# Circuitscape/Circuitscape.jl

Hardware: AMD Instinct MI355X
Metric: pair-solves/sec (AMG-PCG, setup amortised over 100 pairs) on 10000x10000 raster pairwise (higher is better)
Workload: dtype f64

## Files before the change

### circuitscape.jl_amd/csrc/common.h

```cpp
#pragma once
#include <hip/hip_runtime.h>

#include <atomic>
#include <cstdint>
#include <cstdlib>
#include <map>
#include <mutex>
#include <cstdio>
#include <cstring>
#include <stdexcept>
#include <string>
#include <utility>
#include <vector>

#include "../../include/csgpu.h"

namespace csgpu {

struct Error : public std::runtime_error {
  int code;
  Error(int c, const std::string& m) : std::runtime_error(m), code(c) {}
};

#define CS_HIP(expr)                                                                                    \
  do {                                                                                                  \
    hipError_t _e = (expr);                                                                             \
    if (_e != hipSuccess) {                                                                             \
      char _buf[512];                                                                                   \
      snprintf(_buf, sizeof(_buf), "%s failed: %s (%s:%d)", #expr, hipGetErrorString(_e), __FILE__,     \
               __LINE__);                                                                               \
      throw ::csgpu::Error((int)_e == (int)hipErrorOutOfMemory ? CSGPU_OOM : CSGPU_HIP_ERROR, _buf);    \
    }                                                                                                   \
  } while (0)

#define CS_REQUIRE(cond, code, msg)                  \
  do {                                               \
    if (!(cond)) throw ::csgpu::Error((code), (msg)); \
  } while (0)

inline void check_launch(const char* what) {
  hipError_t e = hipGetLastError();
  if (e != hipSuccess) throw Error(CSGPU_HIP_ERROR, std::string(what) + ": " + hipGetErrorString(e));
}

struct Knobs {
  int last_level_sweeps = 0;
  bool enrich = true;
  int enrich_steps = 6;
  double enrich_tau = 0.06;
  int64_t dia25_min_rows = 16384;
  bool dia25_prefetch = true;
  int dia25_waves = 0;
  bool dia25_fused_j0 = true;
  int stream = 0;
  int64_t stream_min = (int64_t)1 << 25;
  double hetero_fp64_frac = 0.03;
  int tail_rows = 4096;
  int poly_lattice = 0;
  double poly_strength = 0.0, poly_coef = 1.0, poly_smin = 8.0, poly_smax = 1000.0;
  bool cellspace = true, cellspace_from_csr = true;
  double cellspace_min_frac = 0.5;
  bool lattice_l1 = true;
  int lattice_l1_min_rows = 16384;
  bool stencil = true, two_product = true;
  bool direct_lattice = true, lattice_s = true, lattice_q = true, direct_tiles = true, tile_pieces = true, direct_at = true;
  double tile_theta = 0.03, tile_split_min = 0.005;
  bool dirichlet_coarse = true, deflation = true, tail_projection = true;
  bool expander_probe = true;
  bool reorder = false;
  int coarse_smoother = 0;
  int nu_l1 = 0, nu_deep = 0;
  int64_t host_stream_block = 0;
  bool wide_csr = false;
  bool fixed_k = false;
  bool recompute_ap = true;
  int fused_restrict = 0;
  int fused_seg = 64;
  int fused_level1 = 0;
  bool sparse_init = true;
  int64_t collapse_min = -1;
  bool longrow = true, narrow_tile = false;
  int spmv_grid_cap = 65536, dia_seg = 0, restrict_seg = 32;
  int verbose = 0;
  double pinv_cut = 0.0;
  bool kernel_gain_ref = false, tail_debug = false;
  bool galerkin_staged = false;
  bool raster_transpose = true;
  bool enrich_fused = true;
  int apq_nt = 256;
  int timed_launches = 512;
};

inline const Knobs*& knobs_slot() {
  static thread_local const Knobs* p = nullptr;
  return p;
}
inline const Knobs& knobs() {
  static const Knobs dflt;
  const Knobs* p = knobs_slot();
  return p ? *p : dflt;
}
struct KnobScope {
  const Knobs* prev;
  explicit KnobScope(const Knobs* k) : prev(knobs_slot()) { knobs_slot() = k; }
  ~KnobScope() { knobs_slot() = prev; }
  KnobScope(const KnobScope&) = delete;
  KnobScope& operator=(const KnobScope&) = delete;
};

static std::atomic<int64_t> g_live_bytes{0};

struct DevicePool {
  static const int kMaxDev = 64;
  struct Blk {
    void* p;
    size_t cap;
    uint64_t seq;
  };
  std::mutex mu[kMaxDev];
  std::multimap<size_t, Blk> ready[kMaxDev];
  std::vector<Blk> pending[kMaxDev];
  size_t pooled[kMaxDev] = {0};
  size_t limit[kMaxDev] = {0};
  std::atomic<uint64_t> seq{0};
  bool enabled = getenv("CSGPU_NO_POOL") == nullptr;
  void promote(int dev) {
    if (pending[dev].empty()) return;
    (void)hipDeviceSynchronize();
    for (const Blk& b : pending[dev]) ready[dev].emplace(b.cap, b);
    pending[dev].clear();
  }
  void* take(int dev, size_t b, size_t* cap) {
    std::lock_guard<std::mutex> lk(mu[dev]);
    for (int pass = 0; pass < 2; ++pass) {
      auto it = ready[dev].lower_bound(b);
      if (it != ready[dev].end() && it->first <= b + b / 8) {
        void* p = it->second.p;
        *cap = it->second.cap;
        ready[dev].erase(it);
        pooled[dev] -= *cap;
        return p;
      }
      if (pass == 0) {
        bool fits = false;
        for (const Blk& q : pending[dev]) fits = fits || (q.cap >= b && q.cap <= b + b / 8);
        if (!fits) break;
        promote(dev);
      }
    }
    return nullptr;
  }
  void give(int dev, size_t cap, void* p) {
    std::vector<void*> victims;
    {
      std::lock_guard<std::mutex> lk(mu[dev]);
      if (limit[dev] == 0) {
        size_t fr = 0, tot = 0;
        const char* e = getenv("CSGPU_POOL_MAX_GB");
        if (e) limit[dev] = (size_t)(atof(e) * 1073741824.0) + 1;
        else {
          int cur = dev;
          (void)hipGetDevice(&cur);
          if (cur != dev) (void)hipSetDevice(dev);
          const bool ok = hipMemGetInfo(&fr, &tot) == hipSuccess && tot > 0;
          if (cur != dev) (void)hipSetDevice(cur);
          limit[dev] = ok ? tot / 10 * 6 : (size_t)64 << 30;
        }
      }
      pending[dev].push_back(Blk{p, cap, ++seq});
      pooled[dev] += cap;
      if (pooled[dev] > limit[dev]) {
        int cur = dev;
        (void)hipGetDevice(&cur);
        if (cur != dev) (void)hipSetDevice(dev);
        promote(dev);
        if (cur != dev) (void)hipSetDevice(cur);
        while (pooled[dev] > limit[dev] && !ready[dev].empty()) {
          auto oldest = ready[dev].begin();
          for (auto it = ready[dev].begin(); it != ready[dev].end(); ++it)
            if (it->second.seq < oldest->second.seq) oldest = it;
          victims.push_back(oldest->second.p);
          pooled[dev] -= oldest->second.cap;
          ready[dev].erase(oldest);
        }
      }
    }
    for (void* v : victims) hipFree(v);
  }
  size_t trim(int dev) {
    size_t freed = 0;
    for (int d = 0; d < kMaxDev; ++d) {
      if (dev >= 0 && d != dev) continue;
      std::vector<void*> victims;
      {
        std::lock_guard<std::mutex> lk(mu[d]);
        for (auto& kv : ready[d]) victims.push_back(kv.second.p);
        for (const Blk& b : pending[d]) victims.push_back(b.p);
        freed += pooled[d];
        ready[d].clear();
        pending[d].clear();
        pooled[d] = 0;
      }
      for (void* p : victims) hipFree(p);
    }
    return freed;
  }
};
inline DevicePool& device_pool() {
  static DevicePool* p = new DevicePool();
  return *p;
}

struct DBuf {
  void* p = nullptr;
  size_t bytes = 0;
  size_t cap = 0;
  int dev = -1;
  DBuf() {}
  explicit DBuf(size_t b) { alloc(b); }
  DBuf(const DBuf&) = delete;
  DBuf& operator=(const DBuf&) = delete;
  DBuf(DBuf&& o) noexcept : p(o.p), bytes(o.bytes), cap(o.cap), dev(o.dev) {
    o.p = nullptr;
    o.bytes = 0;
    o.cap = 0;
  }
  DBuf& operator=(DBuf&& o) noexcept {
    if (this != &o) {
      release();
      p = o.p;
      bytes = o.bytes;
      cap = o.cap;
      dev = o.dev;
      o.p = nullptr;
      o.bytes = 0;
      o.cap = 0;
    }
    return *this;
  }
  ~DBuf() { release(); }
  void alloc(size_t b) {
    release();
    if (b == 0) return;
    CS_HIP(hipGetDevice(&dev));
    DevicePool& pool = device_pool();
    const bool poolable = pool.enabled && dev >= 0 && dev < DevicePool::kMaxDev;
    cap = b;
    if (poolable) p = pool.take(dev, b, &cap);
    if (!p) {
      cap = b;
      hipError_t e = hipMalloc(&p, b);
      if (e != hipSuccess && poolable && pool.trim(dev) > 0) {
        (void)hipGetLastError();
        e = hipMalloc(&p, b);
      }
      if (e != hipSuccess) {
        p = nullptr;
        cap = 0;
        CS_HIP(e);
      }
    }
    bytes = b;
    g_live_bytes += (int64_t)b;
  }
  void release() {
    if (p) {
      DevicePool& pool = device_pool();
      if (pool.enabled && dev >= 0 && dev < DevicePool::kMaxDev)
        pool.give(dev, cap, p);
      else
        hipFree(p);
      g_live_bytes -= (int64_t)bytes;
    }
    p = nullptr;
    bytes = 0;
    cap = 0;
  }
  template <class U>
  U* as() const {
    return (U*)p;
  }
};

template <class U>
inline U* dptr(const DBuf& b) {
  return (U*)b.p;
}

template <class U>
inline DBuf dalloc(size_t count) {
  return DBuf(count * sizeof(U));
}

template <class T>
struct Csr {
  int nrows = 0, ncols = 0;
  int64_t nnz = 0;
  DBuf rowptr, col, val;
  const int* rp() const { return rowptr.as<int>(); }
  const int* ci() const { return col.as<int>(); }
  const T* va() const { return val.as<T>(); }
  int* rp() { return rowptr.as<int>(); }
  int* ci() { return col.as<int>(); }
  T* va() { return val.as<T>(); }
  size_t device_bytes() const { return rowptr.bytes + col.bytes + val.bytes; }
};

template <class T>
struct Dia {
  int64_t n = 0;
  int R = 0;
  DBuf rows;
  const T* data() const { return rows.as<T>(); }
  size_t device_bytes() const { return rows.bytes; }
};

template <class T>
struct LatticeQ {
  int64_t n = 0;
  int R = 0, C = 0, Rc = 0, Cc = 0;
  DBuf q;
  const T* data() const { return q.as<T>(); }
  size_t device_bytes() const { return q.bytes; }
};

inline int ceil_div(int64_t a, int64_t b) { return (int)((a + b - 1) / b); }

static const int kBlock = 256;
static const int kMaxGrid = 2048;
inline int grid_for(int64_t work_items, int per_block = kBlock) {
  int64_t g = (work_items + per_block - 1) / per_block;
  if (g < 1) g = 1;
  if (g > kMaxGrid) g = kMaxGrid;
  return (int)g;
}

}
```

### circuitscape.jl_amd/csrc/csgpu.hip

```cpp
#include <atomic>
#include <chrono>
#include <memory>
#include <mutex>
#include <thread>

#include "currents.h"
#include "pairs.h"
#include "pcg.h"
#include "raster.h"
#include "lattice_setup.h"
#include "reorder.h"

namespace csgpu {

static thread_local std::string g_last_error;

struct GroundedJob {
  const void* rhs = nullptr;
  const int64_t *sptr = nullptr, *sidx = nullptr;
  const void* sval = nullptr;
  const int64_t *gptr = nullptr, *gidx = nullptr;
  const int64_t* check = nullptr;
  void *check_out = nullptr, *x_out = nullptr, *curr_out = nullptr, *cum_inout = nullptr, *max_inout = nullptr;
};
// ... 834 lines not shown
    if (ok) {
      amg_setup_levels(H, sp, nullptr, nullptr, carry, st);
      CS_HIP(hipEventRecord(e1, st));
      CS_HIP(hipEventSynchronize(e1));
      float ms = 0;
      CS_HIP(hipEventElapsedTime(&ms, e0, e1));
      H.setup_ms = ms;
      if constexpr (MIXED) Aouter.nrows = Aouter.ncols = (int)n;
      csr_ready = false;
      if (kn.verbose)
        fprintf(stderr, "csgpu: %lld x %lld raster through the index-free pipeline (%lld rows, %lld nodes, %d levels)\n",
                (long long)R, (long long)C, (long long)n, (long long)n_api, (int)H.levels.size());
    }
    hipEventDestroy(e0);
    hipEventDestroy(e1);
    return ok;
  }

  bool setup_lattice_direct(DBuf& dcond, DBuf& dground, DBuf& node, int64_t R, int64_t C, int four, int avg_res, int reg,
                            std::chrono::steady_clock::time_point t0, int colmajor = 0) {
    const int64_t ncells = R * C;
    const int gc = grid_for(ncells);
    if (cellspace) {
      cellmap.alloc((size_t)ncells * sizeof(int));
      node2cell.alloc((size_t)n_api * sizeof(int));
      cell2node.alloc((size_t)ncells * sizeof(int));
    }
    hipLaunchKernelGGL((raster_maps_kernel<T>), dim3(gc), dim3(256), 0, st, (int)R, (int)C, (const T*)dptr<T>(dcond),
                       (const int*)dptr<int>(node), dptr<int>(nodemap), cellspace ? dptr<int>(cellmap) : (int*)nullptr,
                       cellspace ? dptr<int>(node2cell) : (int*)nullptr, cellspace ? dptr<int>(cell2node) : (int*)nullptr,
                       colmajor);
    dia.n = ncells;
    dia.R = (int)R;
    dia.rows.alloc((size_t)ncells * 5 * sizeof(T));
    if (dground.p) ground_node.alloc((size_t)ncells * sizeof(T));
    DBuf part = dalloc<double>(gc), cnt = dalloc<unsigned long long>(gc), size0;
    hipLaunchKernelGGL((raster_dia_kernel<T>), dim3(gc), dim3(256), 0, st, (int)R, (int)C, four, avg_res,
                       (const T*)dptr<T>(dcond), dground.p ? (const T*)dptr<T>(dground) : (const T*)nullptr, dptr<T>(dia.rows),
                       dground.p ? dptr<T>(ground_node) : (T*)nullptr, dptr<double>(part), dptr<unsigned long long>(cnt),
                       colmajor);
    if (cellspace) size0.alloc((size_t)ncells * sizeof(long long));
    hipLaunchKernelGGL((raster_dia_finish_kernel<T>), dim3(gc), dim3(256), 0, st, (int)R, (int)C, (const T*)dptr<T>(dcond),
                       dptr<T>(dia.rows), (const double*)dptr<double>(part), gc,
                       reg ? (double)std::numeric_limits<T>::epsilon() : 0.0,
                       cellspace ? dptr<long long>(size0) : (long long*)nullptr, colmajor);
    std::vector<unsigned long long> hc((size_t)gc);
    CS_HIP(hipMemcpyAsync(hc.data(), cnt.p, hc.size() * sizeof(unsigned long long), hipMemcpyDeviceToHost, st));
    check_launch("raster -> lattice form");
    CS_HIP(hipStreamSynchronize(st));
    nnz_api = 0;
    for (unsigned long long v : hc) nnz_api += (int64_t)v;
    nnz = nnz_api + (n - n_api);
    dcond.release();
    dground.release();
    node.release();
    upload_ms = std::chrono::duration<double, std::milli>(std::chrono::steady_clock::now() - t0).count();
    if (lattice_pipeline_hierarchy(size0, R, C)) return true;
    CS_REQUIRE(nnz < ((int64_t)1 << 31), CSGPU_BAD_ARGS, "raster too large for the CSR pipeline");
    Csr<T> A;
    dia_to_csr(dia, A, st);
    DBuf drow((size_t)n * sizeof(int)), dcol((size_t)n * sizeof(int));
    hipLaunchKernelGGL(lattice_coords_kernel, dim3(grid_for(n)), dim3(256), 0, st, n, (int)R, dptr<int>(drow), dptr<int>(dcol));
    dia = Dia<T>();
    finish_setup(std::move(A), dptr<int>(drow), dptr<int>(dcol), (int)R,
                 cellspace ? (const long long*)dptr<long long>(size0) : (const long long*)nullptr);
    return true;
  }

  void setup_from_raster(const void* cond, int64_t R, int64_t C, int four, int avg_res, int reg,
                         const void* ground = nullptr) {
    KnobScope ks(&kn);
    auto t0 = std::chrono::steady_clock::now();
    const int64_t ncells = R * C;
    DBuf dcond((size_t)ncells * sizeof(T));
    CS_HIP(hipMemcpyAsync(dcond.p, cond, (size_t)ncells * sizeof(T), hipMemcpyHostToDevice, st));
    DBuf dground;
    if (ground) {
      dground.alloc((size_t)ncells * sizeof(T));
      CS_HIP(hipMemcpyAsync(dground.p, ground, (size_t)ncells * sizeof(T), hipMemcpyHostToDevice, st));
    }
    DBuf node = dalloc<int>((size_t)ncells + 1);
    CS_HIP(hipMemsetAsync(node.p, 0, ((size_t)ncells + 1) * sizeof(int), st));
    const int gc = grid_for(ncells);
    const bool transposed = kn.raster_transpose && R >= 32 && C >= 32;
    DBuf dcondT, dgroundT;
    if (transposed) {
      const int gt = (int)std::min<int64_t>(((R + 31) / 32) * ((C + 31) / 32), 65536);
      dcondT.alloc((size_t)ncells * sizeof(T));
      hipLaunchKernelGGL((raster_transpose_kernel<T>), dim3(gt), dim3(256), 0, st, (int)R, (int)C, (const T*)dptr<T>(dcond),
                         dptr<T>(dcondT));
      if (ground) {
        dgroundT.alloc((size_t)ncells * sizeof(T));
        hipLaunchKernelGGL((raster_transpose_kernel<T>), dim3(gt), dim3(256), 0, st, (int)R, (int)C,
                           (const T*)dptr<T>(dground), dptr<T>(dgroundT));
      }
    }
    hipLaunchKernelGGL((raster_valid_kernel<T>), dim3(gc), dim3(256), 0, st, (int)R, (int)C,
                       transposed ? dptr<T>(dcondT) : dptr<T>(dcond), dptr<int>(node), transposed ? 1 : 0);
    DBuf total = dalloc<int>(1);
    exclusive_scan_i32(dptr<int>(node), ncells + 1, st, dptr<int>(total));
    n_api = read_int(dptr<int>(total), st);
    CS_REQUIRE(n_api > 0, CSGPU_BAD_ARGS, "raster has no cell with positive conductance");
    cellspace = want_cellspace(n_api, ncells, R, C);
    n = cellspace ? ncells : n_api;
    raster_rows = R;
    raster_cols = C;
    nodemap.alloc((size_t)ncells * sizeof(int));
    if (n == ncells && want_lattice_pipeline(R, C)) {
      if (setup_lattice_direct(transposed ? dcondT : dcond, transposed ? dgroundT : dground, node, R, C, four, avg_res, reg, t0,
                               transposed ? 1 : 0))
        return;
    }
    CS_REQUIRE(ncells * 9 < ((int64_t)1 << 31), CSGPU_BAD_ARGS,
               "raster too large for the CSR pipeline (int32 entry offsets); only all-valid / mostly-valid rasters without "
               "polygons, with the default two-product fine level, go through the index-free pipeline");
    if (cellspace) {
      cellmap.alloc((size_t)ncells * sizeof(int));
      node2cell.alloc((size_t)n_api * sizeof(int));
      cell2node.alloc((size_t)ncells * sizeof(int));
    }
    Csr<T> A;
    A.nrows = A.ncols = (int)n;
    A.rowptr.alloc((size_t)(n + 1) * sizeof(int));
    CS_HIP(hipMemsetAsync(A.rp(), 0, (size_t)(n + 1) * sizeof(int), st));
    hipLaunchKernelGGL((raster_count_kernel<T>), dim3(gc), dim3(256), 0, st, (int)R, (int)C, four, dptr<T>(dcond),
                       dptr<int>(node), A.rp(), dptr<int>(nodemap), cellspace ? 1 : 0,
                       cellspace ? dptr<int>(cellmap) : (int*)nullptr, cellspace ? dptr<int>(node2cell) : (int*)nullptr,
                       cellspace ? dptr<int>(cell2node) : (int*)nullptr);
    exclusive_scan_i32(A.rp(), n + 1, st, dptr<int>(total));
    nnz = read_int(dptr<int>(total), st);
    nnz_api = nnz - (n - n_api);
    A.nnz = nnz;
    A.col.alloc((size_t)nnz * sizeof(int));
    A.val.alloc((size_t)nnz * sizeof(T));
    DBuf drow((size_t)n * sizeof(int)), dcol((size_t)n * sizeof(int));
    if (ground) ground_node.alloc((size_t)n * sizeof(T));
    hipLaunchKernelGGL((raster_fill_kernel<T>), dim3(gc), dim3(256), 0, st, (int)R, (int)C, four, avg_res,
                       dptr<T>(dcond), dptr<int>(node), A.rp(), A.ci(), A.va(), dptr<int>(drow), dptr<int>(dcol),
                       ground ? (const T*)dptr<T>(dground) : (const T*)nullptr,
                       ground ? dptr<T>(ground_node) : (T*)nullptr, cellspace ? 1 : 0);
    if (reg) {
      const int g = grid_for(nnz);
      DBuf part = dalloc<double>(g);
      hipLaunchKernelGGL((dot_kernel<T, 1, false>), dim3(g), dim3(256), 0, st, nnz, (const T*)A.va(), (const T*)A.va(),
                         dptr<double>(part), (const T*)nullptr, (const T*)nullptr, (double*)nullptr);
      hipLaunchKernelGGL((add_scalar_kernel<T>), dim3(g), dim3(256), 0, st, nnz, A.va(), dptr<double>(part), g,
                         (double)std::numeric_limits<T>::epsilon());
      CS_HIP(hipStreamSynchronize(st));
    }
    DBuf size0;
    if (cellspace) {
      size0.alloc((size_t)n * sizeof(long long));
      hipLaunchKernelGGL((raster_identity_kernel<T>), dim3(gc), dim3(256), 0, st, (int)R, (int)C, (const T*)dptr<T>(dcond),
                         (const int*)A.rp(), A.va(), dptr<long long>(size0));
    }
    check_launch("raster build");
    CS_HIP(hipStreamSynchronize(st));
    dcond.release();
    node.release();
    upload_ms = std::chrono::duration<double, std::milli>(std::chrono::steady_clock::now() - t0).count();
    finish_setup(std::move(A), dptr<int>(drow), dptr<int>(dcol), n == ncells ? (int)R : -1,
                 cellspace ? (const long long*)dptr<long long>(size0) : (const long long*)nullptr);
    if (cellspace && !(dia.n > 0 && H.levels[0].lattice_two_product()) && kn.verbose)
      fprintf(stderr, "csgpu: cell-space raster without the index-free fine level (CSR kernels on %lld rows)\n", (long long)n);
  }

  bool setup_poly_lattice(const void* cond, const int32_t* polymap, int64_t R, int64_t C, int four, int avg_res, int reg,
                          bool is_fallback) {
    if (is_fallback || kn.poly_lattice < 0 || !want_lattice_pipeline(R, C)) return false;
    if (!kn.cellspace || ground_node.p) return false;
    auto t0 = std::chrono::steady_clock::now();
    const int64_t ncells = R * C;
    const T* hc = (const T*)cond;
    int32_t maxid = 0;
    for (int64_t k = 0; k < ncells; ++k) maxid = std::max(maxid, polymap[k]);
// ... 2003 lines not shown
                        const void* source_val, const int64_t* ground_ptr, const int64_t* ground_idx,
                        const int64_t* check_node, void* check_out, void* x_out, void* curr_out, void* cum_curr_inout,
                        void* max_curr_inout, csgpu_stats* stats) {
  if (!h || !sources_args_ok(nrhs, source_ptr, source_idx, ground_ptr, ground_idx, check_node, check_out)) {
    g_last_error = "bad arguments";
    return CSGPU_BAD_ARGS;
  }
  csgpu::GroundedJob job;
  job.sptr = source_ptr;
  job.sidx = source_idx;
  job.sval = source_val;
  job.gptr = ground_ptr;
  job.gidx = ground_idx;
  job.check = check_node;
  job.check_out = check_out;
  job.x_out = x_out;
  job.curr_out = curr_out;
  job.cum_inout = cum_curr_inout;
  job.max_inout = max_curr_inout;
  return grounded_call(h, job, nrhs, stats);
}

int csgpu_spmv_bench(csgpu_handle* h, int k, int reps, double* avg_ms) {
  CS_API_BEGIN
  if (!h || !avg_ms || reps < 1 || !(k == 1 || k == 2 || k == 4 || k == 8 || k == 16 || k == 32)) {
    g_last_error = "bad arguments";
    return CSGPU_BAD_ARGS;
  }
  *avg_ms = h->solver->spmv_bench(k, reps);
  return CSGPU_OK;
  CS_API_END
}

int csgpu_spmv_host(csgpu_handle* h, const void* x, void* y, int k) {
  CS_API_BEGIN
  if (!h || !x || !y || !(k == 1 || k == 2 || k == 4 || k == 8 || k == 16 || k == 32)) {
    g_last_error = "bad arguments";
    return CSGPU_BAD_ARGS;
  }
  h->solver->spmv_host(x, y, k);
  return CSGPU_OK;
  CS_API_END
}

int csgpu_level_spmv_host(csgpu_handle* h, int lvl, int which, const void* x, void* y, int k, double* dots) {
  CS_API_BEGIN
  if (!h || !x || !y || which < 0 || which > 6 || !(k == 1 || k == 2 || k == 4 || k == 8 || k == 16 || k == 32)) {
    g_last_error = "bad arguments";
    return CSGPU_BAD_ARGS;
  }
  h->solver->level_spmv_host(lvl, which, x, y, k, dots);
  return CSGPU_OK;
  CS_API_END
}

int csgpu_get_level_matrix(const csgpu_handle* h, int lvl, int which, int64_t* nrows, int64_t* ncols, int64_t* nnz,
                           int32_t* rowptr, int32_t* colidx, void* vals) {
  CS_API_BEGIN
  if (!h || which < 0 || which > 5) {
    g_last_error = "bad arguments";
    return CSGPU_BAD_ARGS;
  }
  h->solver->get_level_matrix(lvl, which, nrows, ncols, nnz, rowptr, colidx, vals);
  return CSGPU_OK;
  CS_API_END
}

int csgpu_dia_product_host(csgpu_handle* h, const void* z, const void* p_in, const double* beta, void* p_out, void* y,
                           int k, double* dots) {
  CS_API_BEGIN
  if (!h || !z || !p_in || !beta || !p_out || !y || !(k == 1 || k == 2 || k == 4 || k == 8 || k == 16 || k == 32)) {
    g_last_error = "bad arguments";
    return CSGPU_BAD_ARGS;
  }
  h->solver->dia_product_host(z, p_in, beta, p_out, y, k, dots);
  return CSGPU_OK;
  CS_API_END
}

void csgpu_free(csgpu_handle* h) { delete h; }

int64_t csgpu_trim_memory(int device) { return (int64_t)csgpu::device_pool().trim(device); }

}

struct csgpu_multi {
  std::vector<csgpu_handle*> handles;
  std::vector<int> devices;
  int val_bytes = 8;
  int batch = 8;
  std::vector<double> busy_s;
  std::vector<int64_t> pairs_done;
  ~csgpu_multi() {
    for (csgpu_handle* h : handles) delete h;
  }
};

namespace {

int multi_devices(const int32_t* devices, int ndevices, std::vector<int>& out) {
  const int visible = csgpu_device_count();
  if (visible < 1) {
    g_last_error = "no HIP device visible";
    return CSGPU_HIP_ERROR;
  }
  out.clear();
  if (devices) {
    for (int i = 0; i < ndevices; ++i) {
      if (devices[i] < 0 || devices[i] >= visible) {
        g_last_error = "device ordinal out of range";
        return CSGPU_BAD_ARGS;
      }
      out.push_back(devices[i]);
    }
  } else {
    const int nd = ndevices <= 0 ? visible : std::min(ndevices, visible);
    for (int i = 0; i < nd; ++i) out.push_back(i);
  }
  if (out.empty()) {
    g_last_error = "empty device list";
    return CSGPU_BAD_ARGS;
  }
  return CSGPU_OK;
}

template <class F>
int multi_build(const csgpu_opts* opts, const int32_t* devices, int ndevices, int val_bytes, csgpu_multi** out, F build) {
  std::vector<int> devs;
  int rc = multi_devices(devices, ndevices, devs);
  if (rc) return rc;
  std::unique_ptr<csgpu_multi> m(new csgpu_multi());
  m->devices = devs;
  m->val_bytes = val_bytes;
  csgpu_opts o;
  if (opts) o = *opts; else csgpu_default_opts(&o);
  m->batch = std::max(1, std::min(o.batch, (int)csgpu::kMaxK));
  m->handles.assign(devs.size(), nullptr);
  m->busy_s.assign(devs.size(), 0.0);
  m->pairs_done.assign(devs.size(), 0);
  std::vector<int> codes(devs.size(), CSGPU_OK);
  std::vector<std::string> msgs(devs.size());
  std::vector<std::thread> th;
  for (size_t i = 0; i < devs.size(); ++i)
    th.emplace_back([&, i] {
      csgpu_opts oi = o;
      oi.device = devs[i];
      codes[i] = build(&oi, &m->handles[i]);
      if (codes[i]) msgs[i] = csgpu_last_error();
    });
  for (auto& t : th) t.join();
  for (size_t i = 0; i < devs.size(); ++i)
    if (codes[i]) {
      g_last_error = "device " + std::to_string(devs[i]) + ": " + msgs[i];
      return codes[i];
    }
  *out = m.release();
  return CSGPU_OK;
}

void multi_combine_maps(size_t nd, int64_t n, size_t vb, const std::vector<std::vector<char>>& cum,
                        const std::vector<std::vector<char>>& mx, void* cum_curr_inout, void* max_curr_inout) {
  auto combine = [&](int64_t lo, int64_t hi) {
    for (size_t i = 0; i < nd; ++i) {
      if (cum_curr_inout && !cum[i].empty()) {
        if (vb == 8) {
          double* o = (double*)cum_curr_inout;
// ... 395 lines not shown
```

### circuitscape.jl_amd/lib.py

```python
import ctypes
import os

import numpy as np

_HERE = os.path.dirname(os.path.abspath(__file__))
DEFAULT_LIB = os.path.join(_HERE, "libcsgpu.so")

CSGPU_OK, CSGPU_NOT_CONVERGED, CSGPU_HIP_ERROR, CSGPU_OOM, CSGPU_BAD_ARGS, CSGPU_INTERNAL = range(6)
CRIT_KRYLOV, CRIT_TRUE_RESIDUAL, CRIT_BOTH = 0, 1, 2
AGG_AUTO, AGG_MIS2, AGG_GRID = 0, 1, 2

EXPORTS = [
    "csgpu_device_count", "csgpu_default_opts", "csgpu_setup", "csgpu_raster_setup", "csgpu_get_info",
    "csgpu_solve_pairs", "csgpu_solve_pairs_currents", "csgpu_solve_rhs", "csgpu_solve_grounded", "csgpu_solve_sources", "csgpu_solve_region_pairs", "csgpu_spmv_bench", "csgpu_spmv_host", "csgpu_level_spmv_host",
    "csgpu_get_level_matrix", "csgpu_get_permutation", "csgpu_raster_nodemap", "csgpu_components", "csgpu_raster_setup_grounded", "csgpu_raster_setup_poly",
    "csgpu_solve_raster", "csgpu_dia_product_host",
    "csgpu_multi_setup", "csgpu_multi_raster_setup", "csgpu_multi_solve_pairs", "csgpu_multi_solve_pairs_currents",
    "csgpu_multi_solve_grounded", "csgpu_multi_solve_sources", "csgpu_multi_device_count",
    "csgpu_multi_handle", "csgpu_multi_last_busy", "csgpu_multi_free",
    "csgpu_free", "csgpu_trim_memory", "csgpu_last_error", "csgpu_version",
]


class CsgpuError(RuntimeError):
    def __init__(self, code, msg):
        super().__init__(msg)
        self.code = code


OPTS_INT_FIELDS = ("last_level_sweeps", "enrich", "enrich_steps", "dia25_min_rows", "dia25_prefetch", "dia25_waves",
                   "dia25_fused_j0", "stream", "tail_rows", "poly_lattice", "cellspace", "cellspace_from_csr", "lattice_level1",
                   "lattice_level1_min_rows", "lattice_setup", "lattice_s", "lattice_q", "direct_tiles", "tile_pieces",
                   "direct_at", "dirichlet_coarse", "deflation", "tail_projection", "coarse_smoother", "nu_l1", "nu_deep",
                   "wide_csr", "fixed_k", "recompute_ap", "longrow", "narrow_tile", "spmv_grid_cap", "dia_seg", "restrict_seg",
                   "collapse_min", "verbose", "expander_probe", "fused_restrict", "sparse_init", "fused_level1")
OPTS_DOUBLE_FIELDS = ("enrich_tau", "hetero_fp64_frac", "poly_strength", "poly_coef", "poly_smin", "poly_smax",
                      "cellspace_min_frac", "tile_theta", "tile_split_min")


class Opts(ctypes.Structure):
    _fields_ = [
        ("struct_size", ctypes.c_int32), ("device", ctypes.c_int32), ("max_levels", ctypes.c_int32),
        ("max_coarse", ctypes.c_int32), ("aggregation", ctypes.c_int32), ("nu_pre", ctypes.c_int32),
        ("nu_post", ctypes.c_int32), ("criterion", ctypes.c_int32), ("itmax", ctypes.c_int32),
        ("batch", ctypes.c_int32), ("check_every", ctypes.c_int32), ("nu_coarse", ctypes.c_int32),
        ("theta", ctypes.c_double), ("omega_p", ctypes.c_double), ("omega_s", ctypes.c_double),
        ("rtol", ctypes.c_double), ("atol", ctypes.c_double),
        ("node_row", ctypes.c_void_p), ("node_col", ctypes.c_void_p),
        ("precond_bytes", ctypes.c_int32), ("use_graph", ctypes.c_int32),
        ("two_product", ctypes.c_int32), ("stencil", ctypes.c_int32),
        ("explicit_check", ctypes.c_int32), ("reorder", ctypes.c_int32),
    ] + [(name, ctypes.c_int32) for name in OPTS_INT_FIELDS] + [
        ("stream_min", ctypes.c_int64), ("host_stream_block", ctypes.c_int64),
    ] + [(name, ctypes.c_double) for name in OPTS_DOUBLE_FIELDS]


class Info(ctypes.Structure):
    _fields_ = [
        ("n", ctypes.c_int64), ("nnz", ctypes.c_int64), ("levels", ctypes.c_int32), ("val_bytes", ctypes.c_int32),
        ("precond_bytes", ctypes.c_int32), ("lattice_period", ctypes.c_int32),
        ("operator_complexity", ctypes.c_double), ("grid_complexity", ctypes.c_double),
        ("setup_ms", ctypes.c_double), ("upload_ms", ctypes.c_double), ("device_bytes", ctypes.c_int64),
        ("level_n", ctypes.c_int64 * 32), ("level_nnz", ctypes.c_int64 * 32),
        ("spmv_bytes_fine", ctypes.c_int64), ("bytes_per_iteration", ctypes.c_int64),
        ("level_form", ctypes.c_int32 * 32), ("hierarchy_rebuilt_fp64", ctypes.c_int32),
        ("enrich_vectors", ctypes.c_int32), ("host_blocks", ctypes.c_int32), ("reordered", ctypes.c_int32),
        ("batch_width", ctypes.c_int32), ("stream_mode", ctypes.c_int32), ("tail_first_level", ctypes.c_int32),
        ("last_level_sweeps", ctypes.c_int32), ("coarse_chebyshev", ctypes.c_int32), ("cellspace", ctypes.c_int32),
        ("poly_lattice", ctypes.c_int32), ("enrich_on", ctypes.c_int32), ("enrich_tau", ctypes.c_double),
        ("expander_probe_hit", ctypes.c_int32), ("fused_restrict_solves", ctypes.c_int32), ("virtual_rhs_solves", ctypes.c_int32), ("reserved_info3", ctypes.c_int32),
        ("reorder_ms", ctypes.c_double), ("span_before", ctypes.c_double), ("span_after", ctypes.c_double),
    ]


FORM_CSR, FORM_LATTICE9, FORM_LATTICE25, FORM_TAIL = 0, 1, 2, 3


class Stats(ctypes.Structure):
    _fields_ = [
        ("nrhs", ctypes.c_int32), ("max_iters", ctypes.c_int32), ("total_iters", ctypes.c_int64),
        ("max_relres", ctypes.c_double), ("solve_ms", ctypes.c_double), ("device_ms", ctypes.c_double),
        ("cg_spmv_ms", ctypes.c_double), ("cg_spmv_calls", ctypes.c_int64), ("batch", ctypes.c_int32),
        ("not_converged", ctypes.c_int32), ("graph_launches", ctypes.c_int64),
        ("polished_batches", ctypes.c_int64), ("cg_spmv_bytes", ctypes.c_int64), ("stream_slots", ctypes.c_int64),
        ("resid_ms", ctypes.c_double), ("resid_calls", ctypes.c_int64), ("resid_bytes", ctypes.c_int64),
        ("resid_fused", ctypes.c_int32), ("reserved_stats", ctypes.c_int32),
    ]

    def as_dict(self):
        return {k: getattr(self, k) for k, _ in self._fields_}


_LIB = None
_LIB_PATH = None


def _bind(L):
    vp, i64, i32, dbl = ctypes.c_void_p, ctypes.c_int64, ctypes.c_int, ctypes.c_double
    L.csgpu_device_count.restype = i32
    L.csgpu_default_opts.argtypes = [ctypes.POINTER(Opts)]
    L.csgpu_default_opts.restype = None
    L.csgpu_setup.argtypes = [vp, vp, vp, i64, i64, i32, i32, i32, ctypes.POINTER(Opts), ctypes.POINTER(vp)]
    L.csgpu_raster_setup.argtypes = [vp, i64, i64, i32, i32, i32, i32, ctypes.POINTER(Opts), ctypes.POINTER(vp)]
    L.csgpu_get_info.argtypes = [vp, ctypes.POINTER(Info)]
    L.csgpu_solve_pairs.argtypes = [vp, vp, vp, i64, vp, vp, i64, vp, vp, ctypes.POINTER(Stats)]
    L.csgpu_solve_pairs_currents.argtypes = [vp, vp, vp, i64, vp, vp, vp, vp, vp, vp, vp, ctypes.POINTER(Stats)]
    L.csgpu_solve_rhs.argtypes = [vp, vp, i64, vp, ctypes.POINTER(Stats)]
    L.csgpu_solve_grounded.argtypes = [vp, vp, i64, vp, vp, vp, vp, ctypes.POINTER(Stats)]
    L.csgpu_solve_sources.argtypes = [vp, i64, vp, vp, vp, vp, vp, vp, vp, vp, vp, vp, vp, ctypes.POINTER(Stats)]
    L.csgpu_solve_region_pairs.argtypes = [vp, vp, vp, i64, vp, vp, i64, vp, ctypes.POINTER(Stats)]
    L.csgpu_spmv_bench.argtypes = [vp, i32, i32, ctypes.POINTER(dbl)]
    L.csgpu_spmv_host.argtypes = [vp, vp, vp, i32]
    L.csgpu_level_spmv_host.argtypes = [vp, i32, i32, vp, vp, i32, vp]
    L.csgpu_raster_nodemap.argtypes = [vp, vp, ctypes.POINTER(i64), ctypes.POINTER(i64)]
    L.csgpu_components.argtypes = [vp, vp, ctypes.POINTER(i64)]
    L.csgpu_raster_setup_grounded.argtypes = [vp, vp, i64, i64, i32, i32, i32, i32, ctypes.POINTER(Opts), ctypes.POINTER(vp)]
    L.csgpu_raster_setup_poly.argtypes = [vp, vp, i64, i64, i32, i32, i32, i32, ctypes.POINTER(Opts), ctypes.POINTER(vp)]
    L.csgpu_solve_raster.argtypes = [vp, vp, vp, vp, ctypes.POINTER(Stats)]
    L.csgpu_get_level_matrix.argtypes = [vp, i32, i32, ctypes.POINTER(i64), ctypes.POINTER(i64), ctypes.POINTER(i64),
                                         vp, vp, vp]
    L.csgpu_get_permutation.argtypes = [vp, vp]
    L.csgpu_dia_product_host.argtypes = [vp, vp, vp, vp, vp, vp, i32, vp]
    L.csgpu_multi_setup.argtypes = [vp, vp, vp, i64, i64, i32, i32, i32, ctypes.POINTER(Opts), vp, i32, ctypes.POINTER(vp)]
    L.csgpu_multi_raster_setup.argtypes = [vp, i64, i64, i32, i32, i32, i32, ctypes.POINTER(Opts), vp, i32, ctypes.POINTER(vp)]
    L.csgpu_multi_solve_pairs.argtypes = [vp, vp, vp, i64, vp, i64, vp, vp, ctypes.POINTER(Stats)]
    L.csgpu_multi_solve_pairs_currents.argtypes = [vp, vp, vp, i64, vp, vp, vp, vp, ctypes.POINTER(Stats)]
    L.csgpu_multi_solve_pairs_currents.restype = ctypes.c_int
    L.csgpu_multi_solve_grounded.argtypes = [vp, vp, i64, vp, vp, vp, vp, ctypes.POINTER(Stats)]
    L.csgpu_multi_solve_sources.argtypes = [vp, i64, vp, vp, vp, vp, vp, vp, vp, vp, vp, vp, vp, ctypes.POINTER(Stats)]
    L.csgpu_multi_device_count.argtypes = [vp]
    L.csgpu_multi_handle.argtypes = [vp, i32]
    L.csgpu_multi_handle.restype = vp
    L.csgpu_multi_last_busy.argtypes = [vp, vp, vp]
    L.csgpu_multi_free.argtypes = [vp]
    L.csgpu_multi_free.restype = None
    L.csgpu_free.argtypes = [vp]
    L.csgpu_free.restype = None
    L.csgpu_trim_memory.argtypes = [i32]
    L.csgpu_trim_memory.restype = i64
    L.csgpu_last_error.restype = ctypes.c_char_p
    L.csgpu_version.restype = ctypes.c_char_p
    return L


def load(path=None):
    global _LIB, _LIB_PATH
    path = os.path.abspath(path or DEFAULT_LIB)
    if _LIB is not None and _LIB_PATH == path:
        return _LIB
    if not os.path.exists(path):
        raise CsgpuError(CSGPU_INTERNAL,
                         "HIP extension %s not found: build it with `python -c 'import __graft_entry__ as g; "
                         "g.build()'` (hipcc --offload-arch=gfx950). There is no CPU fallback." % path)
    L = ctypes.CDLL(path)
    for name in EXPORTS:
        if not hasattr(L, name):
            raise CsgpuError(CSGPU_INTERNAL, "%s does not export %s" % (path, name))
    _LIB, _LIB_PATH = _bind(L), path
    return _LIB


def lib():
    return _LIB if _LIB is not None else load()


def loaded_path():
    return _LIB_PATH


def _check(rc):
    if rc != 0:
        raise CsgpuError(rc, (lib().csgpu_last_error() or b"").decode("utf-8", "replace"))


def device_count():
    return lib().csgpu_device_count()


def trim_memory(device=-1):
    return lib().csgpu_trim_memory(device)


def default_opts(**kw):
    o = Opts()
    lib().csgpu_default_opts(ctypes.byref(o))
    for k, v in kw.items():
        if not hasattr(o, k):
            raise TypeError("unknown option %r" % k)
        setattr(o, k, v)
    return o


def _ragged(lists):
    ptr = np.zeros(len(lists) + 1, dtype=np.int64)
    ptr[1:] = np.cumsum([len(q) for q in lists])
    idx = np.ascontiguousarray(np.concatenate([np.asarray(q, dtype=np.int64).ravel() for q in lists])
                               if ptr[-1] > 0 else np.zeros(1, dtype=np.int64))
    return ptr, idx


def _sources_args(dtype, n, sources, grounds, values, check, want_voltages, want_currents, cum, mx):
    sources = [[q] if np.isscalar(q) else list(q) for q in sources]
    nrhs = len(sources)
    assert len(grounds) == nrhs
    sptr, sidx = _ragged(sources)
    gptr, gidx = _ragged(grounds)
    sval = None
    if values is not None:
        values = [[v] if np.isscalar(v) else list(v) for v in values]
        assert [len(v) for v in values] == [len(q) for q in sources]
        sval = np.ascontiguousarray(np.concatenate([np.asarray(v, dtype=dtype) for v in values])
                                    if sptr[-1] > 0 else np.zeros(1, dtype=dtype))
    chk = np.ascontiguousarray(check, dtype=np.int64) if check is not None else None
    assert chk is None or chk.shape == (nrhs,)
    cout = np.zeros(nrhs, dtype=dtype) if chk is not None else None
    X = np.zeros((n, nrhs), dtype=dtype, order="F") if want_voltages else None
    C = np.zeros((n, nrhs), dtype=dtype, order="F") if want_currents else None
    for a in (cum, mx):
        assert a is None or (a.dtype == dtype and a.flags["C_CONTIGUOUS"] and a.shape == (n,))
    ptr = lambda a: a.ctypes.data if a is not None else None
    args = [nrhs, sptr.ctypes.data, sidx.ctypes.data, ptr(sval), gptr.ctypes.data, gidx.ctypes.data, ptr(chk), ptr(cout),
            ptr(X), ptr(C), ptr(cum), ptr(mx)]
    return args, (sptr, sidx, sval, gptr, gidx, chk), cout, X, C


class Handle:

    def __init__(self, ptr, dtype, keepalive=None):
        self._p = ptr
        self.dtype = np.dtype(dtype)
        self._keep = keepalive

    def close(self):
        if self._p:
            lib().csgpu_free(self._p)
            self._p = None

    def __del__(self):
        try:
            self.close()
        except Exception:
            pass

    def __enter__(self):
        return self

    def __exit__(self, *a):
        self.close()

    @property
    def info(self):
        i = Info()
        _check(lib().csgpu_get_info(self._p, ctypes.byref(i)))
        d = {k: getattr(i, k) for k, _ in Info._fields_ if k not in ("level_n", "level_nnz", "level_form")}
        d["level_n"] = [i.level_n[l] for l in range(min(i.levels, 32))]
        d["level_nnz"] = [i.level_nnz[l] for l in range(min(i.levels, 32))]
        d["level_form"] = [i.level_form[l] for l in range(min(i.levels, 32))]
        return d

    def solve_pairs(self, src, dst, gather=None, want_voltages=False):
        src = np.ascontiguousarray(src, dtype=np.int64)
        dst = np.ascontiguousarray(dst, dtype=np.int64)
        npairs = len(src)
# ... 406 lines not shown
```

### include/csgpu.h

```cpp
#ifndef CSGPU_H
#define CSGPU_H

#include <stdint.h>

#ifdef __cplusplus
extern "C" {
#endif

typedef struct csgpu_handle csgpu_handle;

enum {
  CSGPU_OK = 0,
  CSGPU_NOT_CONVERGED = 1,
  CSGPU_HIP_ERROR = 2,
  CSGPU_OOM = 3,
  CSGPU_BAD_ARGS = 4,
  CSGPU_INTERNAL = 5
};

enum { CSGPU_CRIT_KRYLOV = 0, CSGPU_CRIT_TRUE_RESIDUAL = 1, CSGPU_CRIT_BOTH = 2 };

enum { CSGPU_AGG_AUTO = 0, CSGPU_AGG_MIS2 = 1, CSGPU_AGG_GRID = 2 };

typedef struct csgpu_opts {
// ... 143 lines not shown
                int val_bytes, int index_base, const csgpu_opts* opts, csgpu_handle** out);

int csgpu_raster_setup(const void* cond, int64_t nrows, int64_t ncols, int val_bytes, int four_neighbors,
                       int avg_resistances, int reg, const csgpu_opts* opts, csgpu_handle** out);

int csgpu_raster_setup_poly(const void* cond, const int32_t* polymap, int64_t nrows, int64_t ncols, int val_bytes,
                            int four_neighbors, int avg_resistances, int reg, const csgpu_opts* opts,
                            csgpu_handle** out);

int csgpu_raster_setup_grounded(const void* cond, const void* ground, int64_t nrows, int64_t ncols, int val_bytes,
                                int four_neighbors, int avg_resistances, int reg, const csgpu_opts* opts,
                                csgpu_handle** out);

int csgpu_solve_raster(csgpu_handle* h, const void* source, void* curr_out, void* volt_out, csgpu_stats* stats);

int csgpu_raster_nodemap(csgpu_handle* h, int32_t* nodemap_out, int64_t* nrows, int64_t* ncols);

int csgpu_components(csgpu_handle* h, int32_t* component_out, int64_t* ncomponents);

int csgpu_get_info(const csgpu_handle* h, csgpu_info* info);

int csgpu_get_permutation(const csgpu_handle* h, int32_t* perm_out);

int csgpu_solve_pairs(csgpu_handle* h, const int64_t* src, const int64_t* dst, int64_t npairs, void* volt_out,
                      const int64_t* gather_idx, int64_t ngather, void* gathered_out, void* resist_out,
                      csgpu_stats* stats);

int csgpu_solve_pairs_currents(csgpu_handle* h, const int64_t* src, const int64_t* dst, int64_t npairs,
                               const int32_t* weights, void* volt_out, void* curr_out, void* cum_curr_inout,
                               void* max_curr_inout, void* branch_out, void* resist_out, csgpu_stats* stats);

int csgpu_solve_rhs(csgpu_handle* h, const void* rhs, int64_t nrhs, void* x_out, csgpu_stats* stats);

int csgpu_solve_grounded(csgpu_handle* h, const void* rhs, int64_t nrhs, const int64_t* ground_ptr,
                         const int64_t* ground_idx, void* x_out, void* curr_out, csgpu_stats* stats);

int csgpu_solve_sources(csgpu_handle* h, int64_t nrhs, const int64_t* source_ptr, const int64_t* source_idx,
                        const void* source_val, const int64_t* ground_ptr, const int64_t* ground_idx,
                        const int64_t* check_node, void* check_out, void* x_out, void* curr_out, void* cum_curr_inout,
                        void* max_curr_inout, csgpu_stats* stats);

int csgpu_solve_region_pairs(csgpu_handle* h, const int64_t* set_ptr, const int64_t* set_nodes, int64_t nsets,
                             const int64_t* src_set, const int64_t* dst_set, int64_t npairs, double* resistances,
                             csgpu_stats* stats);

int csgpu_spmv_bench(csgpu_handle* h, int k, int reps, double* avg_ms);

int csgpu_spmv_host(csgpu_handle* h, const void* x, void* y, int k);

int csgpu_level_spmv_host(csgpu_handle* h, int lvl, int which, const void* x, void* y, int k, double* dots);

int csgpu_get_level_matrix(const csgpu_handle* h, int lvl, int which, int64_t* nrows, int64_t* ncols, int64_t* nnz,
                           int32_t* rowptr, int32_t* colidx, void* vals);

int csgpu_dia_product_host(csgpu_handle* h, const void* z, const void* p_in, const double* beta, void* p_out, void* y,
                           int k, double* dots);

typedef struct csgpu_multi csgpu_multi;
int csgpu_multi_setup(const void* rowptr, const void* colidx, const void* vals, int64_t n, int64_t nnz, int idx_bytes,
                      int val_bytes, int index_base, const csgpu_opts* opts, const int32_t* devices, int ndevices,
                      csgpu_multi** out);
int csgpu_multi_raster_setup(const void* cond, int64_t nrows, int64_t ncols, int val_bytes, int four_neighbors,
                             int avg_resistances, int reg, const csgpu_opts* opts, const int32_t* devices, int ndevices,
                             csgpu_multi** out);
int csgpu_multi_solve_pairs(csgpu_multi* m, const int64_t* src, const int64_t* dst, int64_t npairs,
                            const int64_t* gather_idx, int64_t ngather, void* gathered_out, void* resist_out,
                            csgpu_stats* stats);
int csgpu_multi_solve_pairs_currents(csgpu_multi* m, const int64_t* src, const int64_t* dst, int64_t npairs,
                                     const int32_t* weights, void* cum_curr_inout, void* max_curr_inout, void* resist_out,
                                     csgpu_stats* stats);
int csgpu_multi_solve_grounded(csgpu_multi* m, const void* rhs, int64_t nrhs, const int64_t* ground_ptr,
                               const int64_t* ground_idx, void* x_out, void* curr_out, csgpu_stats* stats);
int csgpu_multi_solve_sources(csgpu_multi* m, int64_t nrhs, const int64_t* source_ptr, const int64_t* source_idx,
                              const void* source_val, const int64_t* ground_ptr, const int64_t* ground_idx,
                              const int64_t* check_node, void* check_out, void* x_out, void* curr_out,
                              void* cum_curr_inout, void* max_curr_inout, csgpu_stats* stats);
int csgpu_multi_device_count(const csgpu_multi* m);
csgpu_handle* csgpu_multi_handle(csgpu_multi* m, int slot);
int csgpu_multi_last_busy(const csgpu_multi* m, double* busy_s, int64_t* pairs_done);
void csgpu_multi_free(csgpu_multi* m);

void csgpu_free(csgpu_handle* h);
int64_t csgpu_trim_memory(int device);
const char* csgpu_last_error(void);
const char* csgpu_version(void);

#ifdef __cplusplus
}
#endif
#endif
```

Baseline: 51.64.

## Rework device memory pool with segment splitting, coalescing and LRU eviction

```diff
diff --git a/circuitscape.jl_amd/csrc/common.h b/circuitscape.jl_amd/csrc/common.h
--- a/circuitscape.jl_amd/csrc/common.h
+++ b/circuitscape.jl_amd/csrc/common.h
@@ -5,7 +5,10 @@
 #include <cstdint>
 #include <cstdlib>
 #include <map>
+#include <algorithm>
+#include <iterator>
 #include <mutex>
+#include <set>
 #include <cstdio>
 #include <cstring>
 #include <stdexcept>
@@ -112,98 +115,243 @@
 
 struct DevicePool {
   static const int kMaxDev = 64;
-  struct Blk {
-    void* p;
+  static const size_t kAlign = 256;
+  enum State : int { kLive = 0, kPending = 1, kReady = 2 };
+  struct Seg {
     size_t cap;
-    uint64_t seq;
+    char* root;
+    size_t root_size;
+    State state;
+    uint64_t use;
+    uint64_t epoch;
   };
-  std::mutex mu[kMaxDev];
-  std::multimap<size_t, Blk> ready[kMaxDev];
-  std::vector<Blk> pending[kMaxDev];
-  size_t pooled[kMaxDev] = {0};
-  size_t limit[kMaxDev] = {0};
-  std::atomic<uint64_t> seq{0};
+  struct Dev {
+    std::mutex mu;
+    std::map<char*, Seg> segs;
+    std::set<std::pair<size_t, char*>> ready;
+    std::vector<char*> pending;
+    size_t pending_bytes = 0;
+    size_t idle = 0, live = 0;
+    size_t limit = 0, total = 0;
+    uint64_t tick = 0, epoch = 1;
+    size_t fragments = 0;
+    bool over = false;
+    int64_t driver_allocs = 0, driver_alloc_bytes = 0, driver_frees = 0, driver_free_bytes = 0;
+    int64_t hits = 0, hit_bytes = 0, splits = 0;
+  };
+  Dev d[kMaxDev];
   bool enabled = getenv("CSGPU_NO_POOL") == nullptr;
+
+  struct DeviceGuard {
+    int prev;
+    bool switched;
+    explicit DeviceGuard(int dev) : prev(dev), switched(false) {
+      (void)hipGetDevice(&prev);
+      if (prev != dev) switched = hipSetDevice(dev) == hipSuccess;
+    }
+    ~DeviceGuard() {
+      if (switched) (void)hipSetDevice(prev);
+    }
+  };
+  void ensure_limit(int dev) {
+    Dev& D = d[dev];
+    if (D.limit != 0) return;
+    size_t fr = 0, tot = 0;
+    DeviceGuard g(dev);
+    const bool ok = hipMemGetInfo(&fr, &tot) == hipSuccess && tot > 0;
+    D.total = ok ? tot : 0;
+    const char* e = getenv("CSGPU_POOL_MAX_GB");
+    if (e) D.limit = (size_t)(atof(e) * 1073741824.0) + 1;
+    else D.limit = ok ? tot / 10 * 8 : (size_t)64 << 30;
+  }
   void promote(int dev) {
-    if (pending[dev].empty()) return;
-    (void)hipDeviceSynchronize();
-    for (const Blk& b : pending[dev]) ready[dev].emplace(b.cap, b);
-    pending[dev].clear();
+    Dev& D = d[dev];
+    if (D.pending.empty()) return;
+    {
+      DeviceGuard g(dev);
+      (void)hipDeviceSynchronize();
+    }
+    for (char* p : D.pending) {
+      auto it = D.segs.find(p);
+      it->second.state = kReady;
+      D.ready.insert({it->second.cap, p});
+    }
+    D.pending.clear();
+    D.pending_bytes = 0;
+  }
+  bool coalesce(int dev) {
+    Dev& D = d[dev];
+    if (D.fragments == 0) return false;
+    bool merged = false;
+    for (auto it = D.segs.begin(); it != D.segs.end(); ++it) {
+      if (it->second.state != kReady) continue;
+      for (auto nx = std::next(it); nx != D.segs.end() && nx->second.state == kReady && nx->second.root == it->second.root;
+           nx = std::next(it)) {
+        D.ready.erase({nx->second.cap, nx->first});
+        D.ready.erase({it->second.cap, it->first});
+        it->second.cap += nx->second.cap;
+        it->second.use = std::max(it->second.use, nx->second.use);
+        it->second.epoch = std::max(it->second.epoch, nx->second.epoch);
+        D.ready.insert({it->second.cap, it->first});
+        D.segs.erase(nx);
+        --D.fragments;
+        merged = true;
+      }
+    }
+    return merged;
+  }
+  void* hand(Dev& D, std::set<std::pair<size_t, char*>>::iterator rit, size_t need, size_t* cap) {
+    char* p = rit->second;
+    D.ready.erase(rit);
+    Seg& s = D.segs.find(p)->second;
+    if (need < s.cap) {
+      Seg rest = s;
+      rest.cap = s.cap - need;
+      s.cap = need;
+      D.segs.emplace(p + need, rest);
+      D.ready.insert({rest.cap, p + need});
+      ++D.splits;
+      ++D.fragments;
+    }
+    s.state = kLive;
+    s.use = ++D.tick;
+    s.epoch = D.epoch;
+    D.idle -= s.cap;
+    D.live += s.cap;
+    ++D.hits;
+    D.hit_bytes += (int64_t)s.cap;
+    *cap = s.cap;
+    return p;
   }
   void* take(int dev, size_t b, size_t* cap) {
-    std::lock_guard<std::mutex> lk(mu[dev]);
-    for (int pass = 0; pass < 2; ++pass) {
-      auto it = ready[dev].lower_bound(b);
-      if (it != ready[dev].end() && it->first <= b + b / 8) {
-        void* p = it->second.p;
-        *cap = it->second.cap;
-        ready[dev].erase(it);
-        pooled[dev] -= *cap;
-        return p;
-      }
-      if (pass == 0) {
-        bool fits = false;
-        for (const Blk& q : pending[dev]) fits = fits || (q.cap >= b && q.cap <= b + b / 8);
-        if (!fits) break;
+    Dev& D = d[dev];
+    std::vector<std::pair<void*, size_t>> victims;
+    {
+      std::lock_guard<std::mutex> lk(D.mu);
+      ensure_limit(dev);
+      const size_t need = (b + kAlign - 1) / kAlign * kAlign;
+      if (D.live + D.idle + b > D.limit) D.over = true;
+      bool drained = false;
+      for (;;) {
+        auto it = D.ready.lower_bound({b, nullptr});
+        if (it != D.ready.end() && it->first <= b + b / 8) return hand(D, it, it->first, cap);
+        if (!drained) {
+          drained = true;
+          bool fits = D.over && D.pending_bytes >= b;
+          for (size_t i = 0; i < D.pending.size() && !fits; ++i) {
+            const size_t c = D.segs.find(D.pending[i])->second.cap;
+            fits = c >= b && c <= b + b / 8;
+          }
+          if (fits) {
+            promote(dev);
+            continue;
+          }
+        }
+        if (D.over) {
+          if (it != D.ready.end()) return hand(D, it, it->first >= need + kAlign ? need : it->first, cap);
+          if (coalesce(dev)) continue;
+        }
+        break;
+      }
+      if (D.live + D.idle + b > D.limit && D.idle > 0) {
         promote(dev);
-      }
-    }
+        coalesce(dev);
+        std::vector<std::pair<std::pair<int, uint64_t>, char*>> cand;
+        for (const auto& r : D.ready) {
+          const Seg& s = D.segs.find(r.second)->second;
+          if (s.cap == s.root_size) cand.push_back({{s.epoch == D.epoch ? 1 : 0, s.use}, r.second});
+        }
+        std::sort(cand.begin(), cand.end());
+        for (const auto& c : cand) {
+          if (D.live + D.idle + b <= D.limit) break;
+          auto it = D.segs.find(c.second);
+          victims.push_back({(void*)c.second, it->second.cap});
+          D.ready.erase({it->second.cap, c.second});
+          D.idle -= it->second.cap;
+          ++D.driver_frees;
+          D.driver_free_bytes += (int64_t)it->second.cap;
+          D.segs.erase(it);
+        }
+        if (!victims.empty()) ++D.epoch;
+      }
+    }
+    for (auto& v : victims) (void)hipFree(v.first);
     return nullptr;
   }
+  void adopt(int dev, void* p, size_t b) {
+    Dev& D = d[dev];
+    std::lock_guard<std::mutex> lk(D.mu);
+    ++D.driver_allocs;
+    D.driver_alloc_bytes += (int64_t)b;
+    D.live += b;
+    if (enabled) D.segs.emplace((char*)p, Seg{b, (char*)p, b, kLive, ++D.tick, D.epoch});
+  }
   void give(int dev, size_t cap, void* p) {
-    std::vector<void*> victims;
+    Dev& D = d[dev];
     {
-      std::lock_guard<std::mutex> lk(mu[dev]);
-      if (limit[dev] == 0) {
-        size_t fr = 0, tot = 0;
-        const char* e = getenv("CSGPU_POOL_MAX_GB");
-        if (e) limit[dev] = (size_t)(atof(e) * 1073741824.0) + 1;
-        else {
-          int cur = dev;
-          (void)hipGetDevice(&cur);
-          if (cur != dev) (void)hipSetDevice(dev);
-          const bool ok = hipMemGetInfo(&fr, &tot) == hipSuccess && tot > 0;
-          if (cur != dev) (void)hipSetDevice(cur);
-          limit[dev] = ok ? tot / 10 * 6 : (size_t)64 << 30;
-        }
-      }
-      pending[dev].push_back(Blk{p, cap, ++seq});
-      pooled[dev] += cap;
-      if (pooled[dev] > limit[dev]) {
-        int cur = dev;
-        (void)hipGetDevice(&cur);
-        if (cur != dev) (void)hipSetDevice(dev);
-        promote(dev);
-        if (cur != dev) (void)hipSetDevice(cur);
-        while (pooled[dev] > limit[dev] && !ready[dev].empty()) {
-          auto oldest = ready[dev].begin();
-          for (auto it = ready[dev].begin(); it != ready[dev].end(); ++it)
-            if (it->second.seq < oldest->second.seq) oldest = it;
-          victims.push_back(oldest->second.p);
-          pooled[dev] -= oldest->second.cap;
-          ready[dev].erase(oldest);
-        }
-      }
-    }
-    for (void* v : victims) hipFree(v);
+      std::lock_guard<std::mutex> lk(D.mu);
+      D.live -= cap;
+      if (enabled) {
+        Seg& s = D.segs.find((char*)p)->second;
+        s.state = kPending;
+        s.use = ++D.tick;
+        D.pending.push_back((char*)p);
+        D.pending_bytes += cap;
+        D.idle += cap;
+        return;
+      }
+      ++D.driver_frees;
+      D.driver_free_bytes += (int64_t)cap;
+    }
+    (void)hipFree(p);
   }
   size_t trim(int dev) {
     size_t freed = 0;
-    for (int d = 0; d < kMaxDev; ++d) {
-      if (dev >= 0 && d != dev) continue;
+    for (int k = 0; k < kMaxDev; ++k) {
+      if (dev >= 0 && k != dev) continue;
+      Dev& D = d[k];
       std::vector<void*> victims;
       {
-        std::lock_guard<std::mutex> lk(mu[d]);
-        for (auto& kv : ready[d]) victims.push_back(kv.second.p);
-        for (const Blk& b : pending[d]) victims.push_back(b.p);
-        freed += pooled[d];
-        ready[d].clear();
-        pending[d].clear();
-        pooled[d] = 0;
-      }
-      for (void* p : victims) hipFree(p);
+        std::lock_guard<std::mutex> lk(D.mu);
+        if (D.idle == 0) continue;
+        promote(k);
+        coalesce(k);
+        for (auto r = D.ready.begin(); r != D.ready.end();) {
+          auto it = D.segs.find(r->second);
+          if (it->second.cap != it->second.root_size) {
+            ++r;
+            continue;
+          }
+          victims.push_back((void*)r->second);
+          freed += it->second.cap;
+          D.idle -= it->second.cap;
+          ++D.driver_frees;
+          D.driver_free_bytes += (int64_t)it->second.cap;
+          D.segs.erase(it);
+          r = D.ready.erase(r);
+        }
+        D.over = false;
+        if (!victims.empty()) ++D.epoch;
+      }
+      for (void* p : victims) (void)hipFree(p);
     }
     return freed;
+  }
+  void stats(int dev, csgpu_pool_stats_t* o) {
+    Dev& D = d[dev];
+    std::lock_guard<std::mutex> lk(D.mu);
+    o->driver_allocs = D.driver_allocs;
+    o->driver_alloc_bytes = D.driver_alloc_bytes;
+    o->driver_frees = D.driver_frees;
+    o->driver_free_bytes = D.driver_free_bytes;
+    o->hits = D.hits;
+    o->hit_bytes = D.hit_bytes;
+    o->splits = D.splits;
+    o->idle_bytes = (int64_t)D.idle;
+    o->live_bytes = (int64_t)D.live;
+    o->limit_bytes = (int64_t)D.limit;
+    o->device_total_bytes = (int64_t)D.total;
+    o->over_cap = D.over ? 1 : 0;
   }
 };
 inline DevicePool& device_pool() {
@@ -244,13 +392,13 @@
     if (b == 0) return;
     CS_HIP(hipGetDevice(&dev));
     DevicePool& pool = device_pool();
-    const bool poolable = pool.enabled && dev >= 0 && dev < DevicePool::kMaxDev;
+    const bool counted = dev >= 0 && dev < DevicePool::kMaxDev;
     cap = b;
-    if (poolable) p = pool.take(dev, b, &cap);
+    if (counted && pool.enabled) p = pool.take(dev, b, &cap);
     if (!p) {
       cap = b;
       hipError_t e = hipMalloc(&p, b);
-      if (e != hipSuccess && poolable && pool.trim(dev) > 0) {
+      if (e != hipSuccess && counted && pool.enabled && pool.trim(dev) > 0) {
         (void)hipGetLastError();
         e = hipMalloc(&p, b);
       }
@@ -259,15 +407,15 @@
         cap = 0;
         CS_HIP(e);
       }
+      if (counted) pool.adopt(dev, p, b);
     }
     bytes = b;
     g_live_bytes += (int64_t)b;
   }
   void release() {
     if (p) {
-      DevicePool& pool = device_pool();
-      if (pool.enabled && dev >= 0 && dev < DevicePool::kMaxDev)
-        pool.give(dev, cap, p);
+      if (dev >= 0 && dev < DevicePool::kMaxDev)
+        device_pool().give(dev, cap, p);
       else
         hipFree(p);
       g_live_bytes -= (int64_t)bytes;
diff --git a/circuitscape.jl_amd/csrc/csgpu.hip b/circuitscape.jl_amd/csrc/csgpu.hip
--- a/circuitscape.jl_amd/csrc/csgpu.hip
+++ b/circuitscape.jl_amd/csrc/csgpu.hip
@@ -940,15 +940,25 @@
     DBuf node = dalloc<int>((size_t)ncells + 1);
     CS_HIP(hipMemsetAsync(node.p, 0, ((size_t)ncells + 1) * sizeof(int), st));
     const int gc = grid_for(ncells);
-    const bool transposed = kn.raster_transpose && R >= 32 && C >= 32;
+    bool transposed = kn.raster_transpose && R >= 32 && C >= 32;
     DBuf dcondT, dgroundT;
     if (transposed) {
+      try {
+        dcondT.alloc((size_t)ncells * sizeof(T));
+        if (ground) dgroundT.alloc((size_t)ncells * sizeof(T));
+      } catch (const Error& e) {
+        if (e.code != CSGPU_OOM) throw;
+        (void)hipGetLastError();
+        dcondT.release();
+        dgroundT.release();
+        transposed = false;
+      }
+    }
+    if (transposed) {
       const int gt = (int)std::min<int64_t>(((R + 31) / 32) * ((C + 31) / 32), 65536);
-      dcondT.alloc((size_t)ncells * sizeof(T));
       hipLaunchKernelGGL((raster_transpose_kernel<T>), dim3(gt), dim3(256), 0, st, (int)R, (int)C, (const T*)dptr<T>(dcond),
                          dptr<T>(dcondT));
       if (ground) {
-        dgroundT.alloc((size_t)ncells * sizeof(T));
         hipLaunchKernelGGL((raster_transpose_kernel<T>), dim3(gt), dim3(256), 0, st, (int)R, (int)C,
                            (const T*)dptr<T>(dground), dptr<T>(dgroundT));
       }
@@ -3118,6 +3128,15 @@
 
 int64_t csgpu_trim_memory(int device) { return (int64_t)csgpu::device_pool().trim(device); }
 
+int csgpu_pool_stats(int device, csgpu_pool_stats_t* out) {
+  if (!out || device < 0 || device >= csgpu::DevicePool::kMaxDev) {
+    g_last_error = "bad arguments";
+    return CSGPU_BAD_ARGS;
+  }
+  csgpu::device_pool().stats(device, out);
+  return CSGPU_OK;
+}
+
 }
 
 struct csgpu_multi {
diff --git a/circuitscape.jl_amd/lib.py b/circuitscape.jl_amd/lib.py
--- a/circuitscape.jl_amd/lib.py
+++ b/circuitscape.jl_amd/lib.py
@@ -18,7 +18,7 @@
     "csgpu_multi_setup", "csgpu_multi_raster_setup", "csgpu_multi_solve_pairs", "csgpu_multi_solve_pairs_currents",
     "csgpu_multi_solve_grounded", "csgpu_multi_solve_sources", "csgpu_multi_device_count",
     "csgpu_multi_handle", "csgpu_multi_last_busy", "csgpu_multi_free",
-    "csgpu_free", "csgpu_trim_memory", "csgpu_last_error", "csgpu_version",
+    "csgpu_free", "csgpu_trim_memory", "csgpu_pool_stats", "csgpu_last_error", "csgpu_version",
 ]
 
 
@@ -74,6 +74,12 @@
 
 
 FORM_CSR, FORM_LATTICE9, FORM_LATTICE25, FORM_TAIL = 0, 1, 2, 3
+
+
+class PoolStats(ctypes.Structure):
+    _fields_ = [(k, ctypes.c_int64) for k in (
+        "driver_allocs", "driver_alloc_bytes", "driver_frees", "driver_free_bytes", "hits", "hit_bytes", "splits",
+        "idle_bytes", "live_bytes", "limit_bytes", "device_total_bytes", "over_cap")]
 
 
 class Stats(ctypes.Structure):
@@ -138,6 +144,7 @@
     L.csgpu_free.restype = None
     L.csgpu_trim_memory.argtypes = [i32]
     L.csgpu_trim_memory.restype = i64
+    L.csgpu_pool_stats.argtypes = [i32, ctypes.POINTER(PoolStats)]
     L.csgpu_last_error.restype = ctypes.c_char_p
     L.csgpu_version.restype = ctypes.c_char_p
     return L
@@ -179,6 +186,12 @@
 
 def trim_memory(device=-1):
     return lib().csgpu_trim_memory(device)
+
+
+def pool_stats(device=0):
+    st = PoolStats()
+    _check(lib().csgpu_pool_stats(device, ctypes.byref(st)))
+    return {k: getattr(st, k) for k, _ in PoolStats._fields_}
 
 
 def default_opts(**kw):
diff --git a/include/csgpu.h b/include/csgpu.h
--- a/include/csgpu.h
+++ b/include/csgpu.h
@@ -249,6 +249,16 @@
 
 void csgpu_free(csgpu_handle* h);
 int64_t csgpu_trim_memory(int device);
+typedef struct csgpu_pool_stats_t {
+  int64_t driver_allocs, driver_alloc_bytes;
+  int64_t driver_frees, driver_free_bytes;
+  int64_t hits, hit_bytes, splits;
+  int64_t idle_bytes, live_bytes;
+  int64_t limit_bytes;
+  int64_t device_total_bytes;
+  int64_t over_cap;
+} csgpu_pool_stats_t;
+int csgpu_pool_stats(int device, csgpu_pool_stats_t* out);
 const char* csgpu_last_error(void);
 const char* csgpu_version(void);
 
```

Measured after the change: 51.74, median of 6. Within noise of the previous version (+0.2%).
